# mahyarnajibi/SNIPER

Measured on AMD Instinct MI355X. Metric: train chips/sec (512x512, R101), higher is better.
Workload: dtype f16

## Files before the change

### sniper_amd/csrc/nn_ops.hip

```cpp
#include "common.h"
#include <algorithm>

typedef _Float16 half_t;
typedef _Float16 half8 __attribute__((ext_vector_type(8)));

__global__ __launch_bounds__(256) void pack_stem_kernel(const float *__restrict__ x, half_t *__restrict__ out, int N, int C,
                                                        int H, int W, int Hp, int Wp, int pad_t, int pad_l,
                                                        const float *__restrict__ scale, const float *__restrict__ shift) {
  const long total = (long)N * Hp * Wp;
  for (long i = (long)blockIdx.x * blockDim.x + threadIdx.x; i < total; i += (long)gridDim.x * blockDim.x) {
    const int xp = (int)(i % Wp);
    const long t = i / Wp;
    const int yp = (int)(t % Hp), n = (int)(t / Hp);
    const int sy = yp - pad_t, sx = xp - pad_l;
    half_t v[4] = {0, 0, 0, 0};
    if ((unsigned)sy < (unsigned)H && (unsigned)sx < (unsigned)W) {
      for (int c = 0; c < C && c < 4; ++c) {
        float f = x[(((long)n * C + c) * H + sy) * W + sx];
        if (scale) f = f * scale[c] + shift[c];
        v[c] = (half_t)f;
      }
    }
    *reinterpret_cast<uint2 *>(out + i * 4) = *reinterpret_cast<uint2 *>(v);
  }
// ... 990 lines not shown
  for (int j = 0; j < 8; ++j) h[j] = (half_t)v[j];
  *reinterpret_cast<half8 *>(p) = h;
}
template <>
__device__ __forceinline__ void store8<float>(float *p, const float v[8]) {
  *reinterpret_cast<float4 *>(p) = make_float4(v[0], v[1], v[2], v[3]);
  *reinterpret_cast<float4 *>(p + 4) = make_float4(v[4], v[5], v[6], v[7]);
}
template <typename TI, typename TO>
__global__ __launch_bounds__(256) void copy2d_vec8_kernel(const TI *__restrict__ in, TO *__restrict__ out, long total8, int cpr8,
                                                          int in_ld, int out_ld, unsigned fd_mul, unsigned fd_sh) {
  for (long i = (long)blockIdx.x * blockDim.x + threadIdx.x; i < total8; i += (long)gridDim.x * blockDim.x) {
    long r;
    int c;
    if (in_ld == cpr8 * 8 && out_ld == in_ld) { r = 0; c = 0; }
    else if (i < (1l << 31)) { r = (long)(((unsigned long long)__umulhi((unsigned)i, fd_mul) + (unsigned)i) >> fd_sh); c = (int)(i - r * cpr8); }
    else { r = i / cpr8; c = (int)(i - r * cpr8); }
    const size_t si = (in_ld == cpr8 * 8 && out_ld == in_ld) ? (size_t)i * 8 : (size_t)r * in_ld + (size_t)c * 8;
    const size_t di = (in_ld == cpr8 * 8 && out_ld == in_ld) ? (size_t)i * 8 : (size_t)r * out_ld + (size_t)c * 8;
    float v[8];
    load8<TI>(in + si, v);
    store8<TO>(out + di, v);
  }
}
static void fastdiv_make_u32(unsigned d, unsigned &mul, unsigned &sh) {
  unsigned s = 0;
  while ((1ull << s) < d) ++s;
  mul = (unsigned)((((unsigned long long)1 << 32) * (((unsigned long long)1 << s) - d)) / d + 1);
  sh = s;
}

SN_EXPORT int sn_copy2d(const void *in, void *out, long rows, int cols, int in_ld, int out_ld, int in_dtype, int out_dtype,
                        sn_stream_t stream) {
  SN_REQUIRE(in && out && rows > 0 && cols > 0, "sn_copy2d: bad arguments");
  hipStream_t s = sn_stream(stream);
  if (cols % 8 == 0 && (in_ld % 8 == 0 || rows == 1) && (out_ld % 8 == 0 || rows == 1) && ((uintptr_t)in % 16) == 0 &&
      ((uintptr_t)out % 16) == 0) {
    const int cpr8 = cols / 8;
    const long total8 = rows * cpr8;
    if (rows == 1) in_ld = out_ld = cols;
    unsigned mul, sh;
    fastdiv_make_u32((unsigned)cpr8, mul, sh);
    const dim3 g(ew_blocks(total8));
    if (in_dtype == 0 && out_dtype == 0)
      hipLaunchKernelGGL((copy2d_vec8_kernel<half_t, half_t>), g, dim3(256), 0, s, (const half_t *)in, (half_t *)out, total8, cpr8, in_ld, out_ld, mul, sh);
    else if (in_dtype == 0 && out_dtype == 1)
      hipLaunchKernelGGL((copy2d_vec8_kernel<half_t, float>), g, dim3(256), 0, s, (const half_t *)in, (float *)out, total8, cpr8, in_ld, out_ld, mul, sh);
    else if (in_dtype == 1 && out_dtype == 0)
      hipLaunchKernelGGL((copy2d_vec8_kernel<float, half_t>), g, dim3(256), 0, s, (const float *)in, (half_t *)out, total8, cpr8, in_ld, out_ld, mul, sh);
    else
      hipLaunchKernelGGL((copy2d_vec8_kernel<float, float>), g, dim3(256), 0, s, (const float *)in, (float *)out, total8, cpr8, in_ld, out_ld, mul, sh);
    SN_CHECK_LAUNCH();
    return SN_OK;
  }
  const dim3 grid(ew_blocks(rows * cols));
  if (in_dtype == 0 && out_dtype == 0)
    hipLaunchKernelGGL((copy2d_kernel<half_t, half_t>), grid, dim3(256), 0, s, (const half_t *)in, (half_t *)out, rows, cols, in_ld, out_ld);
  else if (in_dtype == 0 && out_dtype == 1)
    hipLaunchKernelGGL((copy2d_kernel<half_t, float>), grid, dim3(256), 0, s, (const half_t *)in, (float *)out, rows, cols, in_ld, out_ld);
  else if (in_dtype == 1 && out_dtype == 0)
    hipLaunchKernelGGL((copy2d_kernel<float, half_t>), grid, dim3(256), 0, s, (const float *)in, (half_t *)out, rows, cols, in_ld, out_ld);
  else
    hipLaunchKernelGGL((copy2d_kernel<float, float>), grid, dim3(256), 0, s, (const float *)in, (float *)out, rows, cols, in_ld, out_ld);
  SN_CHECK_LAUNCH();
  return SN_OK;
}

__global__ __launch_bounds__(256) void softmax_fwd_kernel(const float *__restrict__ x, float *__restrict__ p, long outer, int K,
                                                          long inner) {
  const long total = outer * inner;
  for (long i = (long)blockIdx.x * blockDim.x + threadIdx.x; i < total; i += (long)gridDim.x * blockDim.x) {
    const long o = i / inner, s = i - o * inner;
    const float *xi = x + o * K * inner + s;
    float m = xi[0];
    for (int k = 1; k < K; ++k) m = fmaxf(m, xi[(long)k * inner]);
    float z = 0.f;
    for (int k = 0; k < K; ++k) z += expf(xi[(long)k * inner] - m);
    const float iz = 1.f / z;
    float *pi = p + o * K * inner + s;
    for (int k = 0; k < K; ++k) pi[(long)k * inner] = expf(xi[(long)k * inner] - m) * iz;
  }
}

__global__ __launch_bounds__(256) void count_valid_kernel(const float *__restrict__ label, long n, float ignore,
                                                          int *__restrict__ count) {
  int c = 0;
  for (long i = (long)blockIdx.x * blockDim.x + threadIdx.x; i < n; i += (long)gridDim.x * blockDim.x)
    c += (label[i] != ignore);
#pragma unroll
  for (int off = 32; off > 0; off >>= 1) c += __shfl_xor(c, off, 64);
  if ((threadIdx.x & 63) == 0 && c) atomicAdd(count, c);
}

__global__ __launch_bounds__(256) void softmax_bwd_kernel(const float *__restrict__ p, const float *__restrict__ label,
                                                          float *__restrict__ g, long outer, int K, long inner,
                                                          float ignore, int use_ignore, float grad_scale, int normalize_valid,
                                                          const int *__restrict__ valid_count) {
  const long total = outer * inner;
  float mul = grad_scale;
  if (normalize_valid) {
    const int vc = *valid_count;
    mul = grad_scale / (float)(vc > 1 ? vc : 1);
  }
  for (long i = (long)blockIdx.x * blockDim.x + threadIdx.x; i < total; i += (long)gridDim.x * blockDim.x) {
    const long o = i / inner, s = i - o * inner;
    const float l = label[i];
    const bool ign = use_ignore && l == ignore;
    const int li = (int)l;
    for (int k = 0; k < K; ++k) {
      const long idx = o * K * inner + (long)k * inner + s;
      g[idx] = ign ? 0.f : mul * (p[idx] - (k == li ? 1.f : 0.f));
    }
  }
}

SN_EXPORT int sn_softmax_fwd(const float *x, float *p, long outer, int K, long inner, sn_stream_t stream) {
  SN_REQUIRE(x && p && outer > 0 && K > 0 && inner > 0, "sn_softmax_fwd: bad arguments");
  hipLaunchKernelGGL(softmax_fwd_kernel, dim3(ew_blocks(outer * inner)), dim3(256), 0, sn_stream(stream), x, p, outer, K, inner);
  SN_CHECK_LAUNCH();
  return SN_OK;
}

SN_EXPORT int sn_softmax_output_bwd(const float *p, const float *label, float *grad, long outer, int K, long inner,
                                    float ignore_label, int use_ignore, float grad_scale, int normalize_valid, int *ws,
                                    sn_stream_t stream) {
  SN_REQUIRE(p && label && grad && ws, "sn_softmax_output_bwd: null pointer");
  hipStream_t s = sn_stream(stream);
  if (normalize_valid) {
    SN_HIP(hipMemsetAsync(ws, 0, sizeof(int), s));
    hipLaunchKernelGGL(count_valid_kernel, dim3(ew_blocks(outer * inner)), dim3(256), 0, s, label, outer * inner,
                       use_ignore ? ignore_label : -1e30f, ws);
    SN_CHECK_LAUNCH();
  }
  hipLaunchKernelGGL(softmax_bwd_kernel, dim3(ew_blocks(outer * inner)), dim3(256), 0, s, p, label, grad, outer, K, inner,
                     ignore_label, use_ignore, grad_scale, normalize_valid, ws);
  SN_CHECK_LAUNCH();
  return SN_OK;
}

__global__ __launch_bounds__(256) void smooth_l1_kernel(const float *__restrict__ pred, const float *__restrict__ target,
                                                        const float *__restrict__ weight, float *__restrict__ loss,
                                                        float *__restrict__ dpred, long n, float sigma, float grad_scale) {
  const float s2 = sigma * sigma, th = 1.f / s2;
  for (long i = (long)blockIdx.x * blockDim.x + threadIdx.x; i < n; i += (long)gridDim.x * blockDim.x) {
    const float d = pred[i] - target[i], w = weight[i];
    const float ad = fabsf(d);
    if (loss) loss[i] = w * (ad < th ? 0.5f * s2 * d * d : ad - 0.5f * th);
    if (dpred) dpred[i] = grad_scale * w * (ad < th ? s2 * d : (d > 0.f ? 1.f : (d < 0.f ? -1.f : 0.f)));
  }
}

SN_EXPORT int sn_smooth_l1_loss(const float *pred, const float *target, const float *weight, float *loss, float *dpred,
                                long n, float sigma, float grad_scale, sn_stream_t stream) {
  SN_REQUIRE(pred && target && weight && n > 0, "sn_smooth_l1_loss: bad arguments");
  hipLaunchKernelGGL(smooth_l1_kernel, dim3(ew_blocks(n)), dim3(256), 0, sn_stream(stream), pred, target, weight, loss, dpred,
                     n, sigma, grad_scale);
  SN_CHECK_LAUNCH();
  return SN_OK;
}

__global__ __launch_bounds__(256) void sgd_kernel(float *__restrict__ w32, const float *__restrict__ grad, float *__restrict__ mom,
                                                  half_t *__restrict__ w16, long n, float lr, float wd, float momentum,
                                                  float rescale) {
  for (long i = (long)blockIdx.x * blockDim.x + threadIdx.x; i < n; i += (long)gridDim.x * blockDim.x) {
    const float w = w32[i];
    const float g = rescale * grad[i] + wd * w;
    const float m = momentum * mom[i] - lr * g;
    mom[i] = m;
    const float nw = w + m;
    w32[i] = nw;
    if (w16) w16[i] = (half_t)nw;
  }
}

SN_EXPORT int sn_sgd_mom_update(float *w32, const float *grad, float *mom, void *w16, long n, float lr, float wd,
                                float momentum, float rescale, sn_stream_t stream) {
  SN_REQUIRE(w32 && grad && mom && n >= 0, "sn_sgd_mom_update: bad arguments");
  if (n == 0) return SN_OK;
  hipLaunchKernelGGL(sgd_kernel, dim3(ew_blocks(n)), dim3(256), 0, sn_stream(stream), w32, grad, mom, (half_t *)w16, n, lr, wd,
                     momentum, rescale);
  SN_CHECK_LAUNCH();
  return SN_OK;
}

__global__ __launch_bounds__(256) void sgd_dev_kernel(float *__restrict__ w32, const float *__restrict__ grad,
                                                      float *__restrict__ mom, half_t *__restrict__ w16, long n,
                                                      const float *__restrict__ hyper, float lr_mult, float wd_mult) {
  const float lr = hyper[0] * lr_mult, wd = hyper[1] * wd_mult, momentum = hyper[2], rescale = hyper[3];
  for (long i = (long)blockIdx.x * blockDim.x + threadIdx.x; i < n; i += (long)gridDim.x * blockDim.x) {
    const float w = w32[i];
    const float g = rescale * grad[i] + wd * w;
    const float m = momentum * mom[i] - lr * g;
    mom[i] = m;
    const float nw = w + m;
    w32[i] = nw;
    if (w16) w16[i] = (half_t)nw;
  }
}

__global__ __launch_bounds__(256) void sgd_dev_vec4_kernel(float4 *__restrict__ w32, const float4 *__restrict__ grad,
                                                           float4 *__restrict__ mom, half_t *__restrict__ w16, long n4,
                                                           const float *__restrict__ hyper, float lr_mult, float wd_mult) {
  const float lr = hyper[0] * lr_mult, wd = hyper[1] * wd_mult, momentum = hyper[2], rescale = hyper[3];
  typedef half_t half4 __attribute__((ext_vector_type(4)));
  for (long i = (long)blockIdx.x * blockDim.x + threadIdx.x; i < n4; i += (long)gridDim.x * blockDim.x) {
    const float4 w = w32[i], g4 = grad[i], m4 = mom[i];
    float4 nm, nw;
#define SN_SGD_LANE(f)                                                  \
    {                                                                   \
      const float g = rescale * g4.f + wd * w.f;                        \
      nm.f = momentum * m4.f - lr * g;                                  \
      nw.f = w.f + nm.f;                                                \
    }
    SN_SGD_LANE(x) SN_SGD_LANE(y) SN_SGD_LANE(z) SN_SGD_LANE(w)
#undef SN_SGD_LANE
    mom[i] = nm;
    w32[i] = nw;
    if (w16) {
      half4 h;
      h[0] = (half_t)nw.x; h[1] = (half_t)nw.y; h[2] = (half_t)nw.z; h[3] = (half_t)nw.w;
      *reinterpret_cast<half4 *>(w16 + 4 * i) = h;
    }
  }
}

SN_EXPORT int sn_sgd_mom_update_dev(float *w32, const float *grad, float *mom, void *w16, long n, const float *d_hyper,
                                    float lr_mult, float wd_mult, sn_stream_t stream) {
  SN_REQUIRE(w32 && grad && mom && d_hyper && n >= 0, "sn_sgd_mom_update_dev: bad arguments");
  if (n == 0) return SN_OK;
  auto scalar = [&](long from, long count) {
    hipLaunchKernelGGL(sgd_dev_kernel, dim3(ew_blocks(count)), dim3(256), 0, sn_stream(stream), w32 + from, grad + from,
                       mom + from, w16 ? (half_t *)w16 + from : (half_t *)nullptr, count, d_hyper, lr_mult, wd_mult);
  };
  long head = (long)(((16 - ((uintptr_t)w32 & 15)) & 15) / 4);
  if (head > n) head = n;
  const bool same = (((uintptr_t)(w32 + head) | (uintptr_t)(grad + head) | (uintptr_t)(mom + head)) & 15) == 0 &&
                    (w16 == nullptr || ((uintptr_t)((half_t *)w16 + head) & 7) == 0);
  if (!same) {
    scalar(0, n);
    SN_CHECK_LAUNCH();
    return SN_OK;
  }
  if (head > 0) scalar(0, head);
  const long n4 = (n - head) / 4;
  if (n4 > 0)
    hipLaunchKernelGGL(sgd_dev_vec4_kernel, dim3(ew_blocks(n4)), dim3(256), 0, sn_stream(stream), (float4 *)(w32 + head),
                       (const float4 *)(grad + head), (float4 *)(mom + head), w16 ? (half_t *)w16 + head : (half_t *)nullptr, n4,
                       d_hyper, lr_mult, wd_mult);
  const long done = head + 4 * n4;
  if (done < n) scalar(done, n - done);
  SN_CHECK_LAUNCH();
  return SN_OK;
}

__global__ __launch_bounds__(256) void weight_oti_to_ito_kernel(const float *__restrict__ w, half_t *__restrict__ wt, int O, int T,
                                                                int I, int Opad) {
  const long total = (long)Opad * T * I;
  for (long i = (long)blockIdx.x * blockDim.x + threadIdx.x; i < total; i += (long)gridDim.x * blockDim.x) {
    const int o = (int)(i % Opad);
    const long r = i / Opad;
    const int t = (int)(r % T), ci = (int)(r / T);
    wt[i] = o < O ? (half_t)w[((long)o * T + t) * I + ci] : (half_t)0;
  }
}

SN_EXPORT int sn_weight_transpose(const float *w_oti, void *wt_ito_f16, int O, int T, int I, int O_pad, sn_stream_t stream) {
  SN_REQUIRE(w_oti && wt_ito_f16 && O > 0 && T > 0 && I > 0 && O_pad >= O, "sn_weight_transpose: bad arguments");
  hipLaunchKernelGGL(weight_oti_to_ito_kernel, dim3(ew_blocks((long)O_pad * T * I)), dim3(256), 0, sn_stream(stream), w_oti,
                     (half_t *)wt_ito_f16, O, T, I, O_pad);
  SN_CHECK_LAUNCH();
  return SN_OK;
}

struct WtDesc {
  const float *src;
  half_t *dst;
  int O, T, I, Opad, tile0, tiles_o, tiles_i, pad_;
};
static_assert(sizeof(WtDesc) == 48, "WtDesc layout is part of the C ABI (sn_weight_transpose_batched)");

__global__ __launch_bounds__(256) void weight_transpose_batched_kernel(const WtDesc *__restrict__ desc, int nd) {
  __shared__ float sm[64][65];
  const int tile = blockIdx.x;
  int lo = 0, hi = nd - 1;
  while (lo < hi) {
    const int mid = (lo + hi + 1) >> 1;
    if (desc[mid].tile0 <= tile) lo = mid; else hi = mid - 1;
  }
  const WtDesc d = desc[lo];
  const int local = tile - d.tile0, per_t = d.tiles_o * d.tiles_i;
  const int t = local / per_t, rem = local - t * per_t;
  const int o0 = (rem / d.tiles_i) * 64, i0 = (rem % d.tiles_i) * 64;
  const int c = threadIdx.x & 63, r = threadIdx.x >> 6;
#pragma unroll
  for (int k = 0; k < 16; ++k) {
    const int o = o0 + r + 4 * k, ci = i0 + c;
    sm[r + 4 * k][c] = (o < d.O && ci < d.I) ? d.src[((size_t)o * d.T + t) * d.I + ci] : 0.f;
  }
  __syncthreads();
#pragma unroll
  for (int k = 0; k < 16; ++k) {
    const int ci = i0 + r + 4 * k, o = o0 + c;
    if (ci < d.I && o < d.Opad) d.dst[((size_t)ci * d.T + t) * d.Opad + o] = (half_t)sm[c][r + 4 * k];
  }
}

SN_EXPORT int sn_weight_transpose_batched(const void *desc, int n_desc, int total_tiles, sn_stream_t stream) {
  SN_REQUIRE(desc && n_desc > 0 && total_tiles > 0, "sn_weight_transpose_batched: bad arguments");
  hipLaunchKernelGGL(weight_transpose_batched_kernel, dim3(total_tiles), dim3(256), 0, sn_stream(stream), (const WtDesc *)desc,
                     n_desc);
  SN_CHECK_LAUNCH();
  return SN_OK;
}

__global__ __launch_bounds__(256) void ew_f32_kernel(const float *__restrict__ a, const float *__restrict__ b, float *__restrict__ out,
                                                     long n, int op, float scalar) {
  for (long i = (long)blockIdx.x * blockDim.x + threadIdx.x; i < n; i += (long)gridDim.x * blockDim.x) {
    float v;
    switch (op) {
      case 0: v = a[i] - b[i]; break;
      case 1: v = a[i] + b[i]; break;
      case 2: v = a[i] * b[i]; break;
      case 3: v = a[i] * scalar; break;
      default: v = scalar; break;
    }
    out[i] = v;
  }
}

SN_EXPORT int sn_ew_f32(const float *a, const float *b, float *out, long n, int op, float scalar, sn_stream_t stream) {
  SN_REQUIRE(out && n > 0 && op >= 0 && op <= 4, "sn_ew_f32: bad arguments");
  SN_REQUIRE(op == 4 || a, "sn_ew_f32: null a");
  SN_REQUIRE(op > 2 || b, "sn_ew_f32: null b");
  hipLaunchKernelGGL(ew_f32_kernel, dim3(ew_blocks(n)), dim3(256), 0, sn_stream(stream), a, b, out, n, op, scalar);
  SN_CHECK_LAUNCH();
  return SN_OK;
}

template <typename T>
__global__ __launch_bounds__(256) void bias_grad_kernel(const T *__restrict__ dy, float *__restrict__ db, float *__restrict__ part,
                                                        long rows, int C, int ld, long rows_per_block) {
  const long r0 = (long)blockIdx.y * rows_per_block, r1 = min(rows, r0 + rows_per_block);
  const int c = blockIdx.x * 64 + (threadIdx.x & 63);
  const int rl = threadIdx.x >> 6;
  float s = 0.f;
  if (c < C)
    for (long r = r0 + rl; r < r1; r += 4) s += (float)dy[r * ld + c];
  __shared__ float red[4][64];
  red[rl][threadIdx.x & 63] = s;
  __syncthreads();
  if (rl == 0 && c < C) {
    const float t = (red[0][threadIdx.x] + red[1][threadIdx.x]) + (red[2][threadIdx.x] + red[3][threadIdx.x]);
    if (part) part[(size_t)blockIdx.y * C + c] = t;
    else db[c] += t;
  }
}

__global__ __launch_bounds__(256) void bias_grad_vec8_kernel(const half_t *__restrict__ dy, float *__restrict__ db, float *__restrict__ part,
                                                             long rows, int C, int ld, long rows_per_block) {
  const long r0 = (long)blockIdx.y * rows_per_block, r1 = min(rows, r0 + rows_per_block);
  const int lane = threadIdx.x & 63, rl = threadIdx.x >> 6;
  const int c = (blockIdx.x * 64 + lane) * 8;
  float s[8] = {0.f, 0.f, 0.f, 0.f, 0.f, 0.f, 0.f, 0.f};
  if (c < C) {
    long r = r0 + rl;
    for (; r + 12 < r1; r += 16) {
      half8 v[4];
#pragma unroll
      for (int u = 0; u < 4; ++u) v[u] = *reinterpret_cast<const half8 *>(dy + (r + 4 * u) * ld + c);
#pragma unroll
      for (int u = 0; u < 4; ++u)
#pragma unroll
        for (int j = 0; j < 8; ++j) s[j] += (float)v[u][j];
    }
    for (; r < r1; r += 4) {
      const half8 v = *reinterpret_cast<const half8 *>(dy + r * ld + c);
#pragma unroll
      for (int j = 0; j < 8; ++j) s[j] += (float)v[j];
    }
  }
  __shared__ float red[4][64][9];
#pragma unroll
  for (int j = 0; j < 8; ++j) red[rl][lane][j] = s[j];
  __syncthreads();
  if (rl == 0 && c < C) {
#pragma unroll
// ... 73 lines not shown
```

### sniper_amd/csrc/roi_deform.hip

```cpp
#include "common.h"
#include <type_traits>

#include <stdlib.h>

typedef _Float16 half_t;
typedef _Float16 half8 __attribute__((ext_vector_type(8)));

struct RoiGeom {
  int b;
  float wstart, hstart, sub_w, sub_h, roi_w, roi_h;
};

__device__ __forceinline__ RoiGeom roi_geom(const float *__restrict__ rois, const float *__restrict__ trans, int r, int ph,
                                            int pw, int P, int S, float scale, float trans_std) {
#pragma clang fp contract(off)
  const float *q = rois + (size_t)r * 5;
  RoiGeom g;
  g.b = (int)q[0];
  const float sw = roundf(q[1]) * scale - 0.5f, sh = roundf(q[2]) * scale - 0.5f;
  const float ew = (roundf(q[3]) + 1.f) * scale - 0.5f, eh = (roundf(q[4]) + 1.f) * scale - 0.5f;
  g.roi_w = fmaxf(ew - sw, 0.1f);
  g.roi_h = fmaxf(eh - sh, 0.1f);
  const float bin_w = g.roi_w / (float)P, bin_h = g.roi_h / (float)P;
  g.sub_w = bin_w / (float)S;
// ... 1183 lines not shown
  const int C = output_dim * group_size * group_size;
  const long gz = (long)group_size * group_size * sn_div_up(output_dim, 256);
  SN_REQUIRE(gz <= 65535 && B <= 65535, "sn_psroi_pool_bwd: grid too large");
  hipStream_t s = sn_stream(stream);
  int4 *win = (int4 *)ws;
  hipLaunchKernelGGL(dpsroi_window_kernel, dim3(sn_div_up(R, 4)), dim3(256), 0, s, rois, trans, win, R, H, W, pooled,
                     sample_per_part, spatial_scale, trans_std);
  SN_CHECK_LAUNCH();
  const int tiles = sn_div_up(W, 4) * sn_div_up(H, 4);
  if (group_major)
    hipLaunchKernelGGL(psroi_ps_bwd_data_gm_kernel, dim3(tiles, B, (unsigned)sn_div_up(C, 256)), dim3(256), 0, s, (const half_t *)dout,
                       rois, trans, (const int4 *)win, d_data, d_data_f32, R, H, W, C, pooled, sample_per_part, group_size, output_dim,
                       spatial_scale, trans_std);
  else
    hipLaunchKernelGGL(psroi_ps_bwd_data_kernel, dim3(tiles, B, (unsigned)gz), dim3(256), 0, s, (const half_t *)dout, rois, trans,
                       (const int4 *)win, d_data, d_data_f32, R, H, W, C, pooled, sample_per_part, group_size, output_dim,
                       spatial_scale, trans_std);
  SN_CHECK_LAUNCH();
  if (trans) {
    const long waves = (long)R * pooled * pooled;
    hipLaunchKernelGGL(psroi_ps_bwd_trans_kernel, dim3((unsigned)((waves * 64 + 255) / 256)), dim3(256), 0, s,
                       (const half_t *)dout, (const half_t *)data, rois, trans, d_trans, R, H, W, C, pooled, sample_per_part,
                       group_size, output_dim, spatial_scale, trans_std, group_major ? 1 : 0);
    SN_CHECK_LAUNCH();
  }
  return SN_OK;
}

struct DeformSample {
  bool ok;
  int y0, y1, x0, x1;
  float ly, lx;
};

__device__ __forceinline__ DeformSample deform_sample(float py, float px, int H, int W) {
  DeformSample s;
  s.ok = py >= 0.f && px >= 0.f && py < (float)H && px < (float)W;
  s.y0 = (int)floorf(py);
  s.x0 = (int)floorf(px);
  if (s.y0 >= H - 1) { s.y0 = s.y1 = H - 1; s.ly = 0.f; } else { s.y1 = s.y0 + 1; s.ly = py - (float)s.y0; }
  if (s.x0 >= W - 1) { s.x0 = s.x1 = W - 1; s.lx = 0.f; } else { s.x1 = s.x0 + 1; s.lx = px - (float)s.x0; }
  return s;
}

template <typename TO>
__global__ __launch_bounds__(256) void deform_im2col_kernel(const half_t *__restrict__ data, const TO *__restrict__ offset,
                                                            half_t *__restrict__ col, int N, int H, int W, int C, int Ho, int Wo,
                                                            int KH, int KW, int stride, int pad, int dil, int DG, int off_ps,
                                                            SnDiv d_cpr, SnDiv d_T, SnDiv d_Wo, SnDiv d_Ho, SnDiv d_KW, SnDiv d_cg) {
  const int cpr = C >> 3, T = KH * KW;
  const long total = (long)N * Ho * Wo * T * cpr;
  for (long i = (long)blockIdx.x * blockDim.x + threadIdx.x; i < total; i += (long)gridDim.x * blockDim.x) {
    unsigned chq, tapu, oxu, oyu;
    const unsigned t = sn_divmod((unsigned)i, d_cpr, chq);
    const unsigned m = sn_divmod(t, d_T, tapu);
    const unsigned t2 = sn_divmod(m, d_Wo, oxu);
    const int n = (int)sn_divmod(t2, d_Ho, oyu);
    const int ch = (int)chq * 8, tap = (int)tapu, ox = (int)oxu, oy = (int)oyu;
    const int g = (int)sn_div((unsigned)ch, d_cg), kh = (int)sn_div((unsigned)tap, d_KW), kw = tap - kh * KW;
    const TO *op = offset + (size_t)m * off_ps + g * 2 * T + 2 * tap;
    const float py = (float)(oy * stride - pad + kh * dil) + (float)op[0], px = (float)(ox * stride - pad + kw * dil) + (float)op[1];
    const DeformSample s = deform_sample(py, px, H, W);
    half8 o = {0, 0, 0, 0, 0, 0, 0, 0};
    if (s.ok) {
      const half_t *img = data + (size_t)n * H * W * C + ch;
      const half8 v1 = *reinterpret_cast<const half8 *>(img + ((size_t)s.y0 * W + s.x0) * C);
      const half8 v2 = *reinterpret_cast<const half8 *>(img + ((size_t)s.y0 * W + s.x1) * C);
      const half8 v3 = *reinterpret_cast<const half8 *>(img + ((size_t)s.y1 * W + s.x0) * C);
      const half8 v4 = *reinterpret_cast<const half8 *>(img + ((size_t)s.y1 * W + s.x1) * C);
      const float w1 = (1.f - s.ly) * (1.f - s.lx), w2 = (1.f - s.ly) * s.lx, w3 = s.ly * (1.f - s.lx), w4 = s.ly * s.lx;
#pragma unroll
      for (int j = 0; j < 8; ++j)
        o[j] = (half_t)(w1 * (float)v1[j] + w2 * (float)v2[j] + w3 * (float)v3[j] + w4 * (float)v4[j]);
    }
    *reinterpret_cast<half8 *>(col + i * 8) = o;
  }
}

template <typename TO>
__global__ __launch_bounds__(256) void deform_col2im_offset_kernel(const half_t *__restrict__ dcol, const half_t *__restrict__ data,
                                                                   const TO *__restrict__ offset, TO *__restrict__ d_offset, int N,
                                                                   int H, int W, int C, int Ho, int Wo, int KH, int KW, int stride,
                                                                   int pad, int dil, int DG, int off_ps, SnDiv d_cpr, SnDiv d_T,
                                                                   SnDiv d_Wo, SnDiv d_Ho, SnDiv d_KW, SnDiv d_cg) {
  const int cpr = C >> 3, T = KH * KW, cg = C / DG, lpg = cg >> 3;
  const long total = (long)N * Ho * Wo * T * cpr;
  const long i = (long)blockIdx.x * blockDim.x + threadIdx.x;
  const bool active = i < total;
  const long ii = active ? i : total - 1;
  unsigned chq, tapu, oxu, oyu;
  const unsigned t = sn_divmod((unsigned)ii, d_cpr, chq);
  const unsigned m = sn_divmod(t, d_T, tapu);
  const unsigned t2 = sn_divmod(m, d_Wo, oxu);
  const int n = (int)sn_divmod(t2, d_Ho, oyu);
  const int ch = (int)chq * 8, tap = (int)tapu, ox = (int)oxu, oy = (int)oyu;
  const int g = (int)sn_div((unsigned)ch, d_cg), kh = (int)sn_div((unsigned)tap, d_KW), kw = tap - kh * KW;
  const TO *op = offset + (size_t)m * off_ps + g * 2 * T + 2 * tap;
  const float py = (float)(oy * stride - pad + kh * dil) + (float)op[0], px = (float)(ox * stride - pad + kw * dil) + (float)op[1];
  const DeformSample s = deform_sample(py, px, H, W);
  float gy = 0.f, gx = 0.f;
  if (active && s.ok) {
    const half8 go = *reinterpret_cast<const half8 *>(dcol + ii * 8);
    const size_t base = (size_t)n * H * W * C + ch;
    const half8 v1 = *reinterpret_cast<const half8 *>(data + base + ((size_t)s.y0 * W + s.x0) * C);
    const half8 v2 = *reinterpret_cast<const half8 *>(data + base + ((size_t)s.y0 * W + s.x1) * C);
    const half8 v3 = *reinterpret_cast<const half8 *>(data + base + ((size_t)s.y1 * W + s.x0) * C);
    const half8 v4 = *reinterpret_cast<const half8 *>(data + base + ((size_t)s.y1 * W + s.x1) * C);
#pragma unroll
    for (int j = 0; j < 8; ++j) {
      const float d = (float)go[j];
      const float a = (float)v1[j], b = (float)v2[j], c = (float)v3[j], e = (float)v4[j];
      gy += d * ((1.f - s.lx) * (c - a) + s.lx * (e - b));
      gx += d * ((1.f - s.ly) * (b - a) + s.ly * (e - c));
    }
  }
  for (int off = lpg >> 1; off > 0; off >>= 1) {
    gy += __shfl_xor(gy, off, 64);
    gx += __shfl_xor(gx, off, 64);
  }
  if (active && ((ch >> 3) & (lpg - 1)) == 0) {
    TO *dp = d_offset + (size_t)m * off_ps + g * 2 * T + 2 * tap;
    dp[0] = (TO)gy;
    dp[1] = (TO)gx;
  }
}

template <typename TO>
__global__ __launch_bounds__(256) void deform_col2im_data_mfma_kernel(const half_t *__restrict__ dcol, const TO *__restrict__ offset,
                                                                      void *__restrict__ d_data, int out_f32, int H, int W, int C,
                                                                      int Ho, int Wo, int KH, int KW, int stride, int pad, int dil,
                                                                      int DG, int off_ps, int slabs,
                                                                      const unsigned *__restrict__ dmax_bits) {
  __shared__ __attribute__((aligned(16))) half_t w_hi[16][kListPitch];
  __shared__ __attribute__((aligned(16))) half_t w_lo[16][kListPitch];
  __shared__ __attribute__((aligned(16))) int e_row[kListCap];
  __shared__ int seg_n[4];
  const int tid = threadIdx.x, lane = tid & 63, wave = tid >> 6, nwave = blockDim.x >> 6, nthr = blockDim.x;
  const int fr = lane & 15, kg = lane >> 4;
  const unsigned long long lt = (1ull << lane) - 1ull;
  const int T = KH * KW, cg = C / DG;
  const int tiles_x = (W + 3) >> 2;
  const int x0 = (int)(blockIdx.x % tiles_x) * 4, y0 = (int)(blockIdx.x / tiles_x) * 4;
  const int n = blockIdx.y, g = blockIdx.z / slabs, slab = blockIdx.z - g * slabs;
  const int cl0 = slab * nthr + wave * 64;
  int oy_lo = 0, oy_hi = Ho - 1, ox_lo = 0, ox_hi = Wo - 1;
  if (dmax_bits) {
    const float D = __uint_as_float(*dmax_bits);
    if (D < 1.0e6f) {
      const int Di = (int)ceilf(D) + 1, span = (KH > KW ? KH : KW) - 1;
      auto fdiv = [](int a, int b) { return a >= 0 ? a / b : -((-a + b - 1) / b); };
      oy_lo = max(0, -fdiv(-(y0 - Di + pad - span * dil), stride));
      oy_hi = min(Ho - 1, fdiv(y0 + 3 + Di + pad, stride));
      ox_lo = max(0, -fdiv(-(x0 - Di + pad - span * dil), stride));
      ox_hi = min(Wo - 1, fdiv(x0 + 3 + Di + pad, stride));
    }
  }
  const int wh = max(oy_hi - oy_lo + 1, 0), ww = max(ox_hi - ox_lo + 1, 0);
  const int cand = wh * ww * T, cand_full = Ho * Wo * T;
  floatx4 acc[4];
#pragma unroll
  for (int j = 0; j < 4; ++j) acc[j] = floatx4{0.f, 0.f, 0.f, 0.f};
  int cnt = 0;
  auto flush = [&]() {
    const int kend = (cnt + 31) & ~31;
    for (int i = tid; i < (kend - cnt) * 16; i += nthr) {
      const int e = cnt + i / 16, m = i & 15;
      w_hi[m][e] = (half_t)0;
      w_lo[m][e] = (half_t)0;
      if (m == 0) e_row[e] = 0;
    }
    __syncthreads();
    for (int k0 = 0; k0 < cnt; k0 += 32) {
      const half8 a_hi = *reinterpret_cast<const half8 *>(&w_hi[fr][k0 + kg * 8]);
      const half8 a_lo = *reinterpret_cast<const half8 *>(&w_lo[fr][k0 + kg * 8]);
      const int4 r0 = *reinterpret_cast<const int4 *>(&e_row[k0 + kg * 8]);
      const int4 r1 = *reinterpret_cast<const int4 *>(&e_row[k0 + kg * 8 + 4]);
      const int rows[8] = {r0.x, r0.y, r0.z, r0.w, r1.x, r1.y, r1.z, r1.w};
      half8 bv[4];
#pragma unroll
      for (int j = 0; j < 4; ++j) {
        const int cl = cl0 + j * 16 + fr;
#pragma unroll
// ... 55 lines not shown
      e_row[pos] = n * cand_full + idx;
#pragma unroll
      for (int cy = 0; cy < 4; ++cy)
#pragma unroll
        for (int cx = 0; cx < 4; ++cx) {
          const float w = Wy[cy] * Wx[cx];
          const half_t hi = (half_t)w;
          w_hi[cy * 4 + cx][pos] = hi;
          w_lo[cy * 4 + cx][pos] = (half_t)(w - (float)hi);
        }
    }
    cnt += added;
    __syncthreads();
  }
  flush();
  const int y = y0 + kg;
#pragma unroll
  for (int j = 0; j < 4; ++j) {
    const int cl = cl0 + j * 16 + fr;
    if (cl >= cg || y >= H) continue;
#pragma unroll
    for (int r = 0; r < 4; ++r) {
      const int x = x0 + r;
      if (x >= W) continue;
      const size_t o = (((size_t)n * H + y) * W + x) * C + g * cg + cl;
      if (out_f32) ((float *)d_data)[o] = acc[j][r];
      else ((half_t *)d_data)[o] = (half_t)acc[j][r];
    }
  }
}

SN_EXPORT int sn_deform_im2col(const void *data, const void *offset, void *col, int N, int H, int W, int C, int KH, int KW,
                               int stride, int pad, int dil, int deformable_groups, int offset_pix_stride, int offset_dtype,
                               sn_stream_t stream) {
  SN_REQUIRE(data && offset && col && C % 8 == 0 && deformable_groups > 0 && (C / deformable_groups) % 8 == 0,
             "sn_deform_im2col: bad arguments");
  const int Ho = (H + 2 * pad - dil * (KH - 1) - 1) / stride + 1, Wo = (W + 2 * pad - dil * (KW - 1) - 1) / stride + 1;
  const long total = (long)N * Ho * Wo * KH * KW * (C / 8);
  SN_REQUIRE(total < 2147483647L, "sn_deform_im2col: too many column elements for 32-bit indexing");
  const SnDiv d_cpr = sn_div_make(C / 8), d_T = sn_div_make(KH * KW), d_Wo = sn_div_make(Wo), d_Ho = sn_div_make(Ho),
              d_KW = sn_div_make(KW), d_cg = sn_div_make(C / deformable_groups);
  if (offset_dtype == 0)
    hipLaunchKernelGGL((deform_im2col_kernel<half_t>), dim3((unsigned)blocks_for(total)), dim3(256), 0, sn_stream(stream),
                       (const half_t *)data, (const half_t *)offset, (half_t *)col, N, H, W, C, Ho, Wo, KH, KW, stride, pad, dil,
                       deformable_groups, offset_pix_stride, d_cpr, d_T, d_Wo, d_Ho, d_KW, d_cg);
  else
    hipLaunchKernelGGL((deform_im2col_kernel<float>), dim3((unsigned)blocks_for(total)), dim3(256), 0, sn_stream(stream),
                       (const half_t *)data, (const float *)offset, (half_t *)col, N, H, W, C, Ho, Wo, KH, KW, stride, pad, dil,
                       deformable_groups, offset_pix_stride, d_cpr, d_T, d_Wo, d_Ho, d_KW, d_cg);
  SN_CHECK_LAUNCH();
  return SN_OK;
}

template <typename TO>
__global__ __launch_bounds__(256) void deform_absmax_kernel(const TO *__restrict__ offset, long rows, int cols, int ld,
                                                            unsigned *__restrict__ out) {
  float m = 0.f;
  const long total = rows * cols;
  for (long i = (long)blockIdx.x * blockDim.x + threadIdx.x; i < total; i += (long)gridDim.x * blockDim.x) {
    const long r = i / cols;
    const float v = fabsf((float)offset[r * ld + (i - r * cols)]);
    m = (v > m || v != v) ? (v != v ? INFINITY : v) : m;
  }
  for (int off = 32; off > 0; off >>= 1) m = fmaxf(m, __shfl_xor(m, off, 64));
  __shared__ float wmax[4];
  if ((threadIdx.x & 63) == 0) wmax[threadIdx.x >> 6] = m;
  __syncthreads();
  if (threadIdx.x == 0) {
    const float b = fmaxf(fmaxf(wmax[0], wmax[1]), fmaxf(wmax[2], wmax[3]));
    const unsigned bits = __float_as_uint(b);
    if (bits > *reinterpret_cast<volatile unsigned *>(out)) atomicMax(out, bits);
  }
}

SN_EXPORT int sn_deform_col2im(const void *dcol, const void *data, const void *offset, void *d_data, int d_data_f32,
                               void *d_offset, int N, int H, int W, int C, int KH, int KW, int stride, int pad, int dil,
                               int deformable_groups, int offset_pix_stride, int offset_dtype, void *ws, sn_stream_t stream) {
  SN_REQUIRE(dcol && data && offset && C % 8 == 0 && deformable_groups > 0 && N > 0, "sn_deform_col2im: bad arguments");
  SN_REQUIRE(C % deformable_groups == 0, "sn_deform_col2im: C must be a multiple of the deformable groups");
  const int cg = C / deformable_groups, lpg = cg / 8;
  const int Ho = (H + 2 * pad - dil * (KH - 1) - 1) / stride + 1, Wo = (W + 2 * pad - dil * (KW - 1) - 1) / stride + 1;
  SN_REQUIRE((long)N * Ho * Wo * KH * KW < 2147483647L, "sn_deform_col2im: too many sampling points");
  hipStream_t s = sn_stream(stream);
  if (d_offset) {
    SN_REQUIRE(lpg >= 1 && lpg <= 64 && (lpg & (lpg - 1)) == 0 && cg % 8 == 0,
               "sn_deform_col2im: channels per deformable group / 8 must be a power of two <= 64");
    const long total = (long)N * Ho * Wo * KH * KW * (C / 8);
    SN_REQUIRE(total < 2147483647L - 256, "sn_deform_col2im: too many column elements for 32-bit indexing");
    const SnDiv d_cpr = sn_div_make(C / 8), d_T = sn_div_make(KH * KW), d_Wo = sn_div_make(Wo), d_Ho = sn_div_make(Ho),
                d_KW = sn_div_make(KW), d_cg = sn_div_make(cg);
    if (offset_dtype == 0)
      hipLaunchKernelGGL((deform_col2im_offset_kernel<half_t>), dim3((unsigned)((total + 255) / 256)), dim3(256), 0, s,
                         (const half_t *)dcol, (const half_t *)data, (const half_t *)offset, (half_t *)d_offset, N, H, W, C, Ho, Wo,
                         KH, KW, stride, pad, dil, deformable_groups, offset_pix_stride, d_cpr, d_T, d_Wo, d_Ho, d_KW, d_cg);
    else
      hipLaunchKernelGGL((deform_col2im_offset_kernel<float>), dim3((unsigned)((total + 255) / 256)), dim3(256), 0, s,
                         (const half_t *)dcol, (const half_t *)data, (const float *)offset, (float *)d_offset, N, H, W, C, Ho, Wo,
                         KH, KW, stride, pad, dil, deformable_groups, offset_pix_stride, d_cpr, d_T, d_Wo, d_Ho, d_KW, d_cg);
    SN_CHECK_LAUNCH();
  }
  if (d_data) {
    const int bt = cg >= 256 ? 256 : sn_div_up(cg, 64) * 64, slabs = sn_div_up(cg, bt);
    const dim3 grid(sn_div_up(W, 4) * sn_div_up(H, 4), N, deformable_groups * slabs);
    unsigned *dmax = (unsigned *)ws;
    if (dmax) {
      SN_HIP(hipMemsetAsync(dmax, 0, sizeof(unsigned), s));
      const long rows = (long)N * Ho * Wo;
      const int cols = 2 * KH * KW * deformable_groups;
      const long want = (rows * cols + 255) / 256;
      const unsigned blocks = (unsigned)(want > 256 ? 256 : (want < 1 ? 1 : want));
      if (offset_dtype == 0)
        hipLaunchKernelGGL((deform_absmax_kernel<half_t>), dim3(blocks), dim3(256), 0, s, (const half_t *)offset, rows, cols,
                           offset_pix_stride, dmax);
      else
        hipLaunchKernelGGL((deform_absmax_kernel<float>), dim3(blocks), dim3(256), 0, s, (const float *)offset, rows, cols,
                           offset_pix_stride, dmax);
      SN_CHECK_LAUNCH();
    }
    if (offset_dtype == 0)
      hipLaunchKernelGGL((deform_col2im_data_mfma_kernel<half_t>), grid, dim3(bt), 0, s, (const half_t *)dcol,
                         (const half_t *)offset, d_data, d_data_f32, H, W, C, Ho, Wo, KH, KW, stride, pad, dil, deformable_groups,
                         offset_pix_stride, slabs, (const unsigned *)dmax);
    else
      hipLaunchKernelGGL((deform_col2im_data_mfma_kernel<float>), grid, dim3(bt), 0, s, (const half_t *)dcol,
                         (const float *)offset, d_data, d_data_f32, H, W, C, Ho, Wo, KH, KW, stride, pad, dil, deformable_groups,
                         offset_pix_stride, slabs, (const unsigned *)dmax);
    SN_CHECK_LAUNCH();
  }
  return SN_OK;
}
```

Baseline: 988.5.

## Vectorize softmax, valid-count, weight transpose and fuse deform offset absmax

Adds an LDS-staged row softmax forward for inner==1, a float4 row-wise softmax backward, and a two-stage valid-label count with 1024-thread blocks and float4 loads that replaces global atomics. It also vectorizes the batched weight transpose loads and stores, and folds the deformable offset absmax into the col2im offset kernel so a separate pass is skipped. The aim is fewer memory transactions, fewer launches and less atomic contention. The cost is more code paths with alignment conditions, and the count kernel borrows the grad buffer as scratch.

```diff
diff --git a/sniper_amd/csrc/nn_ops.hip b/sniper_amd/csrc/nn_ops.hip
--- a/sniper_amd/csrc/nn_ops.hip
+++ b/sniper_amd/csrc/nn_ops.hip
@@ -1096,14 +1096,105 @@
   }
 }
 
-__global__ __launch_bounds__(256) void count_valid_kernel(const float *__restrict__ label, long n, float ignore,
-                                                          int *__restrict__ count) {
+constexpr int kSmRows = 64;
+constexpr int kSmMaxLdsBytes = 48 * 1024;
+static int softmax_rows_pitch(int K) { return K | 1; }
+static bool softmax_rows_ok(const void *a, const void *b, long outer, int K, long inner) {
+  return inner == 1 && (size_t)kSmRows * softmax_rows_pitch(K) * sizeof(float) <= (size_t)kSmMaxLdsBytes &&
+         outer * K < 2147483647L && ((uintptr_t)a % 16) == 0 && ((uintptr_t)b % 16) == 0;
+}
+
+template <bool TO_LDS>
+__device__ __forceinline__ void softmax_rows_move(float *__restrict__ g, float *__restrict__ sm, int n, int K, int pitch) {
+  const int nv = n >> 2;
+  for (int v = threadIdx.x; v < nv; v += kSmRows) {
+    const int e = v * 4;
+    int row = e / K, k = e - row * K;
+    float4 q;
+    if (TO_LDS) q = *reinterpret_cast<const float4 *>(g + e);
+    float *qe = reinterpret_cast<float *>(&q);
+#pragma unroll
+    for (int j = 0; j < 4; ++j) {
+      if (TO_LDS) sm[row * pitch + k] = qe[j];
+      else qe[j] = sm[row * pitch + k];
+      if (++k == K) { k = 0; ++row; }
+    }
+    if (!TO_LDS) *reinterpret_cast<float4 *>(g + e) = q;
+  }
+  for (int e = nv * 4 + threadIdx.x; e < n; e += kSmRows) {
+    const int row = e / K, k = e - row * K;
+    if (TO_LDS) sm[row * pitch + k] = g[e];
+    else g[e] = sm[row * pitch + k];
+  }
+}
+
+__global__ __launch_bounds__(kSmRows) void softmax_fwd_rows_kernel(const float *__restrict__ x, float *__restrict__ p, int outer,
+                                                                   int K, int pitch) {
+  extern __shared__ float sm_rows[];
+  const int row0 = blockIdx.x * kSmRows, rows = min(kSmRows, outer - row0);
+  const size_t base = (size_t)row0 * K;
+  softmax_rows_move<true>(const_cast<float *>(x) + base, sm_rows, rows * K, K, pitch);
+  __syncthreads();
+  if ((int)threadIdx.x < rows) {
+    float *xi = sm_rows + threadIdx.x * pitch;
+    float m = xi[0];
+    for (int k = 1; k < K; ++k) m = fmaxf(m, xi[k]);
+    float z = 0.f;
+    for (int k = 0; k < K; ++k) z += expf(xi[k] - m);
+    const float iz = 1.f / z;
+    for (int k = 0; k < K; ++k) xi[k] = expf(xi[k] - m) * iz;
+  }
+  __syncthreads();
+  softmax_rows_move<false>(p + base, sm_rows, rows * K, K, pitch);
+}
+
+constexpr int kCountThreads = 1024;
+constexpr long kCountOneBlock = 1L << 19;
+constexpr long kCountPerBlock = 1L << 16;
+
+__device__ __forceinline__ void count_block_store(int c, int *__restrict__ out) {
+  __shared__ int wsum[kCountThreads / 64];
+#pragma unroll
+  for (int off = 32; off > 0; off >>= 1) c += __shfl_xor(c, off, 64);
+  if ((threadIdx.x & 63) == 0) wsum[threadIdx.x >> 6] = c;
+  __syncthreads();
+  if (threadIdx.x < 64) {
+    int t = threadIdx.x < kCountThreads / 64 ? wsum[threadIdx.x] : 0;
+#pragma unroll
+    for (int off = 8; off > 0; off >>= 1) t += __shfl_xor(t, off, 64);
+    if (threadIdx.x == 0) *out = t;
+  }
+}
+
+__global__ __launch_bounds__(kCountThreads) void count_valid_kernel(const float *__restrict__ label, long n, long per_block,
+                                                                    float ignore, int *__restrict__ out) {
+  const long i0 = (long)blockIdx.x * per_block, i1 = min(n, i0 + per_block);
   int c = 0;
-  for (long i = (long)blockIdx.x * blockDim.x + threadIdx.x; i < n; i += (long)gridDim.x * blockDim.x)
-    c += (label[i] != ignore);
-#pragma unroll
-  for (int off = 32; off > 0; off >>= 1) c += __shfl_xor(c, off, 64);
-  if ((threadIdx.x & 63) == 0 && c) atomicAdd(count, c);
+  long i = i0 + threadIdx.x;
+  const long head = min(i1, i0 + (long)(((16 - ((uintptr_t)(label + i0) & 15)) & 15) >> 2));
+  if (i < head) c += (label[i] != ignore);
+  const long nv = (i1 - head) >> 2;
+  const float4 *lv = reinterpret_cast<const float4 *>(label + head);
+  long v = threadIdx.x;
+  for (; v + 7 * kCountThreads < nv; v += 8 * kCountThreads) {
+    float4 q[8];
+#pragma unroll
+    for (int u = 0; u < 8; ++u) q[u] = lv[v + u * kCountThreads];
+#pragma unroll
+    for (int u = 0; u < 8; ++u) c += (q[u].x != ignore) + (q[u].y != ignore) + (q[u].z != ignore) + (q[u].w != ignore);
+  }
+  for (; v < nv; v += kCountThreads) {
+    const float4 q = lv[v];
+    c += (q.x != ignore) + (q.y != ignore) + (q.z != ignore) + (q.w != ignore);
+  }
+  for (i = head + nv * 4 + threadIdx.x; i < i1; i += kCountThreads) c += (label[i] != ignore);
+  count_block_store(c, out + blockIdx.x);
+}
+
+__global__ __launch_bounds__(kCountThreads) void count_sum_kernel(const int *__restrict__ part, int nblk, int *__restrict__ out) {
+  int c = 0;
+  for (int i = threadIdx.x; i < nblk; i += kCountThreads) c += part[i];
+  count_block_store(c, out);
 }
 
 __global__ __launch_bounds__(256) void softmax_bwd_kernel(const float *__restrict__ p, const float *__restrict__ label,
@@ -1128,9 +1219,51 @@
   }
 }
 
+__global__ __launch_bounds__(256) void softmax_bwd_rows_kernel(const float *__restrict__ p, const float *__restrict__ label,
+                                                               float *__restrict__ g, int total, int K, float ignore,
+                                                               int use_ignore, float grad_scale, int normalize_valid,
+                                                               const int *__restrict__ valid_count) {
+  float mul = grad_scale;
+  if (normalize_valid) {
+    const int vc = *valid_count;
+    mul = grad_scale / (float)(vc > 1 ? vc : 1);
+  }
+  const int nv = total >> 2;
+  for (int v = blockIdx.x * blockDim.x + threadIdx.x; v < nv; v += gridDim.x * blockDim.x) {
+    const int e = v * 4;
+    int row = e / K, k = e - row * K;
+    const float4 q = *reinterpret_cast<const float4 *>(p + e);
+    const float *qe = reinterpret_cast<const float *>(&q);
+    float4 out;
+    float *oe = reinterpret_cast<float *>(&out);
+    float l = label[row];
+#pragma unroll
+    for (int j = 0; j < 4; ++j) {
+      const bool ign = use_ignore && l == ignore;
+      const int li = (int)l;
+      oe[j] = ign ? 0.f : mul * (qe[j] - (k == li ? 1.f : 0.f));
+      if (++k == K && e + j + 1 < total) { k = 0; l = label[++row]; }
+    }
+    *reinterpret_cast<float4 *>(g + e) = out;
+  }
+  if (blockIdx.x == 0 && (int)threadIdx.x < total - nv * 4) {
+    const int e = nv * 4 + threadIdx.x, row = e / K, k = e - row * K;
+    const float l = label[row];
+    const bool ign = use_ignore && l == ignore;
+    const int li = (int)l;
+    g[e] = ign ? 0.f : mul * (p[e] - (k == li ? 1.f : 0.f));
+  }
+}
+
 SN_EXPORT int sn_softmax_fwd(const float *x, float *p, long outer, int K, long inner, sn_stream_t stream) {
   SN_REQUIRE(x && p && outer > 0 && K > 0 && inner > 0, "sn_softmax_fwd: bad arguments");
-  hipLaunchKernelGGL(softmax_fwd_kernel, dim3(ew_blocks(outer * inner)), dim3(256), 0, sn_stream(stream), x, p, outer, K, inner);
+  if (softmax_rows_ok(x, p, outer, K, inner)) {
+    const int pitch = softmax_rows_pitch(K);
+    hipLaunchKernelGGL(softmax_fwd_rows_kernel, dim3((unsigned)((outer + kSmRows - 1) / kSmRows)), dim3(kSmRows),
+                       (size_t)kSmRows * pitch * sizeof(float), sn_stream(stream), x, p, (int)outer, K, pitch);
+  } else {
+    hipLaunchKernelGGL(softmax_fwd_kernel, dim3(ew_blocks(outer * inner)), dim3(256), 0, sn_stream(stream), x, p, outer, K, inner);
+  }
   SN_CHECK_LAUNCH();
   return SN_OK;
 }
@@ -1141,13 +1274,26 @@
   SN_REQUIRE(p && label && grad && ws, "sn_softmax_output_bwd: null pointer");
   hipStream_t s = sn_stream(stream);
   if (normalize_valid) {
-    SN_HIP(hipMemsetAsync(ws, 0, sizeof(int), s));
-    hipLaunchKernelGGL(count_valid_kernel, dim3(ew_blocks(outer * inner)), dim3(256), 0, s, label, outer * inner,
-                       use_ignore ? ignore_label : -1e30f, ws);
-    SN_CHECK_LAUNCH();
-  }
-  hipLaunchKernelGGL(softmax_bwd_kernel, dim3(ew_blocks(outer * inner)), dim3(256), 0, s, p, label, grad, outer, K, inner,
-                     ignore_label, use_ignore, grad_scale, normalize_valid, ws);
+    const long n = outer * inner;
+    const float ign = use_ignore ? ignore_label : -1e30f;
+    const long nblk = (n + kCountPerBlock - 1) / kCountPerBlock;
+    if (n <= kCountOneBlock || grad == p) {
+      hipLaunchKernelGGL(count_valid_kernel, dim3(1), dim3(kCountThreads), 0, s, label, n, n, ign, ws);
+      SN_CHECK_LAUNCH();
+    } else {
+      hipLaunchKernelGGL(count_valid_kernel, dim3((unsigned)nblk), dim3(kCountThreads), 0, s, label, n, kCountPerBlock, ign,
+                         (int *)grad);
+      SN_CHECK_LAUNCH();
+      hipLaunchKernelGGL(count_sum_kernel, dim3(1), dim3(kCountThreads), 0, s, (const int *)grad, (int)nblk, ws);
+      SN_CHECK_LAUNCH();
+    }
+  }
+  if (inner == 1 && outer * K < 2147483647L && ((uintptr_t)p % 16) == 0 && ((uintptr_t)grad % 16) == 0)
+    hipLaunchKernelGGL(softmax_bwd_rows_kernel, dim3(ew_blocks((outer * K + 3) / 4)), dim3(256), 0, s, p, label, grad,
+                       (int)(outer * K), K, ignore_label, use_ignore, grad_scale, normalize_valid, ws);
+  else
+    hipLaunchKernelGGL(softmax_bwd_kernel, dim3(ew_blocks(outer * inner)), dim3(256), 0, s, p, label, grad, outer, K, inner,
+                       ignore_label, use_ignore, grad_scale, normalize_valid, ws);
   SN_CHECK_LAUNCH();
   return SN_OK;
 }
@@ -1306,16 +1452,44 @@
   const int t = local / per_t, rem = local - t * per_t;
   const int o0 = (rem / d.tiles_i) * 64, i0 = (rem % d.tiles_i) * 64;
   const int c = threadIdx.x & 63, r = threadIdx.x >> 6;
-#pragma unroll
-  for (int k = 0; k < 16; ++k) {
-    const int o = o0 + r + 4 * k, ci = i0 + c;
-    sm[r + 4 * k][c] = (o < d.O && ci < d.I) ? d.src[((size_t)o * d.T + t) * d.I + ci] : 0.f;
+  if ((d.I & 3) == 0 && ((uintptr_t)d.src & 15) == 0) {
+    const int c4 = (threadIdx.x & 15) * 4, r4 = threadIdx.x >> 4;
+#pragma unroll
+    for (int k = 0; k < 4; ++k) {
+      const int o = o0 + r4 + 16 * k, ci = i0 + c4;
+      const float4 q = (o < d.O && ci < d.I) ? *reinterpret_cast<const float4 *>(d.src + ((size_t)o * d.T + t) * d.I + ci)
+                                             : float4{0.f, 0.f, 0.f, 0.f};
+      sm[r4 + 16 * k][c4] = q.x;
+      sm[r4 + 16 * k][c4 + 1] = q.y;
+      sm[r4 + 16 * k][c4 + 2] = q.z;
+      sm[r4 + 16 * k][c4 + 3] = q.w;
+    }
+  } else {
+#pragma unroll
+    for (int k = 0; k < 16; ++k) {
+      const int o = o0 + r + 4 * k, ci = i0 + c;
+      sm[r + 4 * k][c] = (o < d.O && ci < d.I) ? d.src[((size_t)o * d.T + t) * d.I + ci] : 0.f;
+    }
   }
   __syncthreads();
-#pragma unroll
-  for (int k = 0; k < 16; ++k) {
-    const int ci = i0 + r + 4 * k, o = o0 + c;
-    if (ci < d.I && o < d.Opad) d.dst[((size_t)ci * d.T + t) * d.Opad + o] = (half_t)sm[c][r + 4 * k];
+  if ((d.Opad & 7) == 0 && ((uintptr_t)d.dst & 15) == 0) {
+    const int o8 = (threadIdx.x & 7) * 8, r8 = threadIdx.x >> 3;
+#pragma unroll
+    for (int k = 0; k < 2; ++k) {
+      const int ci = i0 + r8 + 32 * k, o = o0 + o8;
+      if (ci < d.I && o < d.Opad) {
+        half8 h;
+#pragma unroll
+        for (int j = 0; j < 8; ++j) h[j] = (half_t)sm[o8 + j][r8 + 32 * k];
+        *reinterpret_cast<half8 *>(d.dst + ((size_t)ci * d.T + t) * d.Opad + o) = h;
+      }
+    }
+  } else {
+#pragma unroll
+    for (int k = 0; k < 16; ++k) {
+      const int ci = i0 + r + 4 * k, o = o0 + c;
+      if (ci < d.I && o < d.Opad) d.dst[((size_t)ci * d.T + t) * d.Opad + o] = (half_t)sm[c][r + 4 * k];
+    }
   }
 }
 
diff --git a/sniper_amd/csrc/roi_deform.hip b/sniper_amd/csrc/roi_deform.hip
--- a/sniper_amd/csrc/roi_deform.hip
+++ b/sniper_amd/csrc/roi_deform.hip
@@ -1289,7 +1289,8 @@
                                                                    const TO *__restrict__ offset, TO *__restrict__ d_offset, int N,
                                                                    int H, int W, int C, int Ho, int Wo, int KH, int KW, int stride,
                                                                    int pad, int dil, int DG, int off_ps, SnDiv d_cpr, SnDiv d_T,
-                                                                   SnDiv d_Wo, SnDiv d_Ho, SnDiv d_KW, SnDiv d_cg) {
+                                                                   SnDiv d_Wo, SnDiv d_Ho, SnDiv d_KW, SnDiv d_cg,
+                                                                   unsigned *__restrict__ dmax_out) {
   const int cpr = C >> 3, T = KH * KW, cg = C / DG, lpg = cg >> 3;
   const long total = (long)N * Ho * Wo * T * cpr;
   const long i = (long)blockIdx.x * blockDim.x + threadIdx.x;
@@ -1305,6 +1306,18 @@
   const TO *op = offset + (size_t)m * off_ps + g * 2 * T + 2 * tap;
   const float py = (float)(oy * stride - pad + kh * dil) + (float)op[0], px = (float)(ox * stride - pad + kw * dil) + (float)op[1];
   const DeformSample s = deform_sample(py, px, H, W);
+  if (dmax_out) {
+    const float v0 = fabsf((float)op[0]), v1 = fabsf((float)op[1]);
+    float mx = (v0 != v0 || v1 != v1) ? INFINITY : fmaxf(v0, v1);
+    for (int off = 32; off > 0; off >>= 1) mx = fmaxf(mx, __shfl_xor(mx, off, 64));
+    __shared__ float wmax[4];
+    if ((threadIdx.x & 63) == 0) wmax[threadIdx.x >> 6] = mx;
+    __syncthreads();
+    if (threadIdx.x == 0) {
+      const unsigned bits = __float_as_uint(fmaxf(fmaxf(wmax[0], wmax[1]), fmaxf(wmax[2], wmax[3])));
+      if (bits > *reinterpret_cast<volatile unsigned *>(dmax_out)) atomicMax(dmax_out, bits);
+    }
+  }
   float gy = 0.f, gx = 0.f;
   if (active && s.ok) {
     const half8 go = *reinterpret_cast<const half8 *>(dcol + ii * 8);
@@ -1526,6 +1539,8 @@
   const int Ho = (H + 2 * pad - dil * (KH - 1) - 1) / stride + 1, Wo = (W + 2 * pad - dil * (KW - 1) - 1) / stride + 1;
   SN_REQUIRE((long)N * Ho * Wo * KH * KW < 2147483647L, "sn_deform_col2im: too many sampling points");
   hipStream_t s = sn_stream(stream);
+  unsigned *dmax = d_data ? (unsigned *)ws : nullptr;
+  if (dmax) SN_HIP(hipMemsetAsync(dmax, 0, sizeof(unsigned), s));
   if (d_offset) {
     SN_REQUIRE(lpg >= 1 && lpg <= 64 && (lpg & (lpg - 1)) == 0 && cg % 8 == 0,
                "sn_deform_col2im: channels per deformable group / 8 must be a power of two <= 64");
@@ -1536,19 +1551,17 @@
     if (offset_dtype == 0)
       hipLaunchKernelGGL((deform_col2im_offset_kernel<half_t>), dim3((unsigned)((total + 255) / 256)), dim3(256), 0, s,
                          (const half_t *)dcol, (const half_t *)data, (const half_t *)offset, (half_t *)d_offset, N, H, W, C, Ho, Wo,
-                         KH, KW, stride, pad, dil, deformable_groups, offset_pix_stride, d_cpr, d_T, d_Wo, d_Ho, d_KW, d_cg);
+                         KH, KW, stride, pad, dil, deformable_groups, offset_pix_stride, d_cpr, d_T, d_Wo, d_Ho, d_KW, d_cg, dmax);
     else
       hipLaunchKernelGGL((deform_col2im_offset_kernel<float>), dim3((unsigned)((total + 255) / 256)), dim3(256), 0, s,
                          (const half_t *)dcol, (const half_t *)data, (const float *)offset, (float *)d_offset, N, H, W, C, Ho, Wo,
-                         KH, KW, stride, pad, dil, deformable_groups, offset_pix_stride, d_cpr, d_T, d_Wo, d_Ho, d_KW, d_cg);
+                         KH, KW, stride, pad, dil, deformable_groups, offset_pix_stride, d_cpr, d_T, d_Wo, d_Ho, d_KW, d_cg, dmax);
     SN_CHECK_LAUNCH();
   }
   if (d_data) {
     const int bt = cg >= 256 ? 256 : sn_div_up(cg, 64) * 64, slabs = sn_div_up(cg, bt);
     const dim3 grid(sn_div_up(W, 4) * sn_div_up(H, 4), N, deformable_groups * slabs);
-    unsigned *dmax = (unsigned *)ws;
-    if (dmax) {
-      SN_HIP(hipMemsetAsync(dmax, 0, sizeof(unsigned), s));
+    if (dmax && !d_offset) {
       const long rows = (long)N * Ho * Wo;
       const int cols = 2 * KH * KW * deformable_groups;
       const long want = (rows * cols + 255) / 256;
```

New measurement: 987.9. Within noise of the previous version (-0.1%).
